# mbavaro/gnss-sdr.ru

Measured on NVIDIA B200. Metric: tracking channel*Msamples/s, higher is better.
Workload: dtype int32

## Files before the change

gnss_sdr_ru_b200/csrc/track_seg.cuh:

```cuda
#pragma once
#include "track_common.cuh"

struct __align__(16) BlockParams {
  uint32_t cph0, kph0, cinc, kinc;
  uint32_t hc0, w1, stale_idx, stale_bits;
  int mode, event;
  uint32_t wtot;
  uint32_t seg;
  double dinv;
  uint32_t kseg;
  uint32_t pad;
};
static_assert(sizeof(BlockParams) == 64, "BlockParams: four 16-byte rows");

#ifndef SEG_U2
#define SEG_U2 1
#endif
#ifndef SEG_PIN
#define SEG_PIN 0
#endif

__device__ __forceinline__ uint32_t lds_u32(uint32_t addr) {
  uint32_t t;
  asm volatile("ld.shared.u32 %0, [%1];" : "=r"(t) : "r"(addr));
  return t;
}

__device__ __forceinline__ bool seg_kinc_ok(uint32_t kinc) { return kinc >= (1u << 29) && 7ull * kinc <= (1ull << 32); }
__device__ __forceinline__ bool seg_kinc_ok16(uint32_t kinc) { return kinc >= (1u << 28) && 15ull * kinc <= (1ull << 32); }

__device__ __forceinline__ uint32_t seg_start(uint32_t m, double nk05 , double dinv) {
  const double x = fma((double)m, 4294967296.0, nk05);
  return (uint32_t)(x * dinv) + 1u;
}

struct SegBounds {
  uint32_t tile_lo, tile_hi, bits_lo, bits_hi, vlut_lo, vlut_hi;
};
template <int H>
__device__ __forceinline__ void correlate_segments(uint32_t q, uint32_t cph, uint32_t ks, const uint32_t cinc, const uint32_t kinc,
                                                   const uint32_t k7, const uint32_t hp, const int nvalid, const uint32_t vlut_lane,
                                                   const PipeK K, int &accE, int &accP, int &accL, const SegBounds bnd,
                                                   const uint32_t kseg_addr ,
                                                   const uint32_t kconst_addr ) {
  int aE = 0, aP = 0, aL = 0;
  TCHECK(0, ks < kinc || nvalid == 0);
  TCHECK(1, hp >= bnd.bits_lo && hp + 4u * (H + 1) <= bnd.bits_hi + 4u);
  uint32_t a0 = (q >> 3) & ~3u;
  TCHECK(2, a0 >= bnd.tile_lo && a0 + 8u <= bnd.tile_hi);
  uint32_t lo = lds_u32(a0), hi = lds_u32(a0 + 4);
  uint32_t t = lds_u32(hp);
  uint32_t hq = hp;
  const uint32_t hq_valid = hp + 4u * (uint32_t)nvalid;
  const uint32_t hq_end = hp + 4u * (uint32_t)H;
#if SEG_PIN
  uint32_t k7r, k1r, k2048r;
  asm volatile("ld.volatile.shared.u32 %0, [%1];" : "=r"(k7r) : "r"(kseg_addr));
  asm volatile("ld.volatile.shared.v2.u32 {%0, %1}, [%2];" : "=r"(k1r), "=r"(k2048r) : "r"(kconst_addr));
  TCHECK(0, k7r == k7 && k1r == K.k1 && k2048r == K.k2048);
#else
  const uint32_t k7r = k7, k1r = K.k1, k2048r = K.k2048;
#endif
#define SEG_BODY(tc, tn)                                                                                             \
  {                                                                                                                  \
                      \
    const uint32_t wd = __funnelshift_r(lo, hi, q);                                                                  \
            \
    uint32_t u, c;                                                                                                   \
    asm("add.cc.u32 %0, %2, %3;\n\taddc.u32 %1, 0, 0;" : "=r"(u), "=r"(c) : "r"(ks), "r"(k7r));                    \
    const uint32_t e8 = k1r - c;                                                                                     \
    ks = e8 * kinc + u;                                                                                              \
    q = e8 * 4u + (q + 28u);                                                                                         \
     \
    const uint32_t a = (q >> 3) & ~3u;                                                                               \
    TCHECK(2, a >= bnd.tile_lo && a + 8u <= bnd.tile_hi);    \
    lo = lds_u32(a);                                                                                                 \
    hi = lds_u32(a + 4);                                                                                             \
    tn = lds_u32(hq + 4u);                                                                                           \
    int v[8];                                                                                                        \
    _Pragma("unroll") for (int k = 0; k < 8; k++) {                                                                  \
                                                          \
      uint32_t sh;                                                                                                   \
      if (k == 0)                                                                                                    \
        sh = wd << 7;                                                                                                \
      else if (k == 1)                                                                                               \
        sh = wd << 3;                                                                                                \
      else                                                                                                           \
        sh = wd >> (4 * k - 7);                                                                                      \
      uint32_t ca;                                                                                                   \
      asm("lop3.b32 %0, %1, 0x780, %2, 0xEA;" : "=r"(ca) : "r"(sh), "r"(vlut_lane));   \
      const uint32_t eaddr = (cph >> 29) * k2048r + ca;            \
      TCHECK(3, eaddr >= bnd.vlut_lo && eaddr + 4u <= bnd.vlut_hi);                           \
      v[k] = (int)lds_u32(eaddr);                                                                                    \
      if (k < 7) cph += cinc;                                                                                        \
    }                                                                                                                \
    cph = e8 * cinc + cph;                                                                                           \
    const int S = (int)e8 * v[7] + (((v[0] + v[1] + v[2]) + (v[3] + v[4] + v[5])) + v[6]);                           \
    if (hq < hq_valid) {                                                                                             \
      aE += sext8(tc, 0) * S;                                                                                        \
      aP += sext8(tc, 1) * S;                                                                                        \
      aL += sext8(tc, 2) * S;                                                                                        \
    }                                                                                                                \
    hq += 4u;                                                                                                        \
  }
#if SEG_U2
  uint32_t t2;
  if (H & 1) {
    SEG_BODY(t, t2)
    t = t2;
  }
  if (H > 1) {
#pragma unroll 1
    do {
      SEG_BODY(t, t2)
      SEG_BODY(t2, t)
    } while (hq != hq_end);
  }
#else
#pragma unroll 1
  do {
    uint32_t t_next;
    SEG_BODY(t, t_next)
    t = t_next;
  } while (hq != hq_end);
#endif
#undef SEG_BODY
  accE = aE;
  accP = aP;
  accL = aL;
}

template <int H>
__device__ __forceinline__ void correlate_segments_i8(uint32_t q, uint32_t cph, uint32_t ks, const uint32_t cinc, const uint32_t kinc,
                                                      const uint32_t k7, const uint32_t hp, const int nvalid, const uint32_t lut_addr,
                                                      const PipeK K, int &accE, int &accP, int &accL, const SegBounds bnd) {
  static_assert(8 * H * 384 <= 32767, "int8 segment run: a 16-bit lane of the packed sums can overflow");
  int aE = 0, aP = 0, aL = 0;
  TCHECK(0, ks < kinc || nvalid == 0);
  TCHECK(1, hp >= bnd.bits_lo && hp + 4u * (H + 1) <= bnd.bits_hi + 4u);
  uint32_t hq = hp;
  const uint32_t hq_valid = hp + 4u * (uint32_t)nvalid;
  const uint32_t hq_end = hp + 4u * (uint32_t)H;
#pragma unroll 1
  do {
    const uint32_t a = (q >> 3) & ~3u;
    TCHECK(2, a >= bnd.tile_lo && a + 20u <= bnd.tile_hi);
    uint32_t w[5];
#pragma unroll
    for (int i = 0; i < 5; i++) w[i] = lds_u32(a + 4u * i);
    const uint32_t t = lds_u32(hq);
    uint32_t x[4];
#pragma unroll
    for (int i = 0; i < 4; i++) x[i] = __funnelshift_r(w[i], w[i + 1], q);
    uint32_t u, c;
    asm("add.cc.u32 %0, %2, %3;\n\taddc.u32 %1, 0, 0;" : "=r"(u), "=r"(c) : "r"(ks), "r"(k7));
    const uint32_t e8 = K.k1 - c;
    ks = e8 * kinc + u;
    q = e8 * 16u + (q + 112u);
    int v[8];
#pragma unroll
    for (int k = 0; k < 8; k++) {
      const int I = sext8(x[k >> 1], (k & 1) * 2), Q = sext8(x[k >> 1], (k & 1) * 2 + 1);
      uint32_t lx, ly;
      asm volatile("ld.shared.v2.u32 {%0, %1}, [%2];" : "=r"(lx), "=r"(ly) : "r"((cph >> 29) * K.k8 + lut_addr));
      v[k] = I * (int)lx + Q * (int)ly;
      if (k < 7) cph += cinc;
    }
    cph = e8 * cinc + cph;
    const int S = (int)e8 * v[7] + (((v[0] + v[1] + v[2]) + (v[3] + v[4] + v[5])) + v[6]);
    if (hq < hq_valid) {
      aE += sext8(t, 0) * S;
      aP += sext8(t, 1) * S;
      aL += sext8(t, 2) * S;
    }
    hq += 4u;
  } while (hq != hq_end);
  accE = aE;
  accP = aP;
  accL = aL;
}

template <int H>
__device__ __forceinline__ void correlate_segments16(uint32_t q, uint32_t cph, uint32_t ks, const uint32_t cinc, const uint32_t kinc,
                                                     const uint32_t k15, const uint32_t hp, const int nvalid, const uint32_t vlut_lane,
                                                     const PipeK K, int &accE, int &accP, int &accL, const SegBounds bnd) {
  int aE = 0, aP = 0, aL = 0;
  TCHECK(0, ks < kinc || nvalid == 0);
  TCHECK(1, hp >= bnd.bits_lo && hp + 4u * (H + 1) <= bnd.bits_hi + 4u);
  uint32_t hq = hp;
  const uint32_t hq_valid = hp + 4u * (uint32_t)nvalid;
  const uint32_t hq_end = hp + 4u * (uint32_t)H;
#pragma unroll 1
  do {
    const uint32_t a = (q >> 3) & ~3u;
    TCHECK(2, a >= bnd.tile_lo && a + 12u <= bnd.tile_hi);
    const uint32_t w0 = lds_u32(a), w1 = lds_u32(a + 4), w2 = lds_u32(a + 8);
    const uint32_t t = lds_u32(hq);
    const uint32_t wd[2] = {__funnelshift_r(w0, w1, q), __funnelshift_r(w1, w2, q)};
    uint32_t u, c;
    asm("add.cc.u32 %0, %2, %3;\n\taddc.u32 %1, 0, 0;" : "=r"(u), "=r"(c) : "r"(ks), "r"(k15));
    const uint32_t e16 = K.k1 - c;
    ks = e16 * kinc + u;
    q = e16 * 4u + (q + 60u);
    int S = 0;
#pragma unroll
    for (int half = 0; half < 2; half++) {
      int v[8];
#pragma unroll
      for (int k = 0; k < 8; k++) {
        uint32_t sh;
        if (k == 0)
          sh = wd[half] << 7;
        else if (k == 1)
          sh = wd[half] << 3;
        else
          sh = wd[half] >> (4 * k - 7);
        uint32_t ca;
        asm("lop3.b32 %0, %1, 0x780, %2, 0xEA;" : "=r"(ca) : "r"(sh), "r"(vlut_lane));
        const uint32_t eaddr = (cph >> 29) * K.k2048 + ca;
        TCHECK(3, eaddr >= bnd.vlut_lo && eaddr + 4u <= bnd.vlut_hi);
        v[k] = (int)lds_u32(eaddr);
        if (half == 0 || k < 7) cph += cinc;
      }
      S += ((v[0] + v[1] + v[2]) + (v[3] + v[4] + v[5])) + v[6] + (half == 0 ? v[7] : (int)e16 * v[7]);
    }
    cph = e16 * cinc + cph;
    if (hq < hq_valid) {
      aE += sext8(t, 0) * S;
      aP += sext8(t, 1) * S;
      aL += sext8(t, 2) * S;
    }
    hq += 4u;
  } while (hq != hq_end);
  accE = aE;
  accP = aP;
  accL = aL;
}

struct SampleCtx {
  uint32_t cph0, kph0, cinc, kinc, hc0, w1, stale_idx;
  const uint8_t *tile;
  const uint32_t *tbl;
  const uint2 *lut;
  int fmt;
};
__device__ __forceinline__ void eval_sample(const SampleCtx &c, int i, int (&sumA)[6], int (&sumB)[6], bool &anyB) {
  const unsigned long long ki = (unsigned long long)c.kph0 + (unsigned long long)i * c.kinc;
  const uint32_t wb = (uint32_t)(ki >> 32);
  const bool inA = wb < c.w1;
  const uint32_t rel = wb - c.w1;
  const uint32_t hh = inA ? c.hc0 + wb : (rel == 0 ? c.stale_idx : rel);
  TCHECK(5, hh < SMEM_TBL);
  const uint32_t t = c.tbl[hh];
  int I, Q;
  load_sample(c.tile, c.fmt, i, I, Q);
  const uint2 ab = c.lut[(c.cph0 + (uint32_t)i * c.cinc) >> 29];
  const int v = I * (int)ab.x + Q * (int)ab.y;
  int vi, vq;
  unpack_lanes(v, vi, vq);
  const int cE = sext8(t, 0), cP = sext8(t, 1), cL = sext8(t, 2);
  if (inA) {
    sumA[0] += cL * vi; sumA[1] += cL * vq; sumA[2] += cP * vi;
    sumA[3] += cP * vq; sumA[4] += cE * vi; sumA[5] += cE * vq;
  } else {
    sumB[0] += cL * vi; sumB[1] += cL * vq; sumB[2] += cP * vi;
    sumB[3] += cP * vq; sumB[4] += cE * vi; sumB[5] += cE * vq;
    anyB = true;
  }
}

template <int NT, int H, int SLOTS = 8, bool I8 = false>
__device__ __forceinline__ void seg_block(const BlockParams &p, const SampleCtx &sc, const uint32_t tile_addr, const uint32_t tbl_addr,
                                          const uint32_t alias_addr, const uint32_t vlut_lane, const PipeK K, const int nsamp,
                                          const int ptid, int (&sumA)[6], int (&sumB)[6], bool &anyB, const SegBounds bnd_in,
                                          const uint32_t kseg_addr = 0, const uint32_t kconst_addr = 0) {
  constexpr int STEP = NT == 96 ? 7 : 1;
  const int tid = (ptid * STEP) % NT;
  const uint32_t wtot = p.wtot, w1 = p.w1;
  const uint32_t NF = wtot > 0 ? wtot - 1 : 0;
  constexpr uint32_t OWNED = (uint32_t)(NT - 1) * H;
  const double nk05 = -(double)p.kph0 - 0.5;
  uint32_t m0, nv;
  if (tid < NT - 1) {
    const uint32_t first = (uint32_t)tid * H;
    m0 = 1 + first;
    nv = NF > first ? min(NF - first, (uint32_t)H) : 0u;
    if (m0 < w1 && w1 < m0 + nv) nv = w1 - m0;
  } else {
    m0 = 1;
    nv = 0;
    if (w1 >= 2) {
      const uint32_t ts = (w1 - 2) / H, first = ts * H;
      const uint32_t end = 1 + first + (NF > first ? min(NF - first, (uint32_t)H) : 0u);
      if (ts < (uint32_t)(NT - 1) && w1 < end) {
        m0 = w1;
        nv = end - w1;
      }
    }
  }
  if (nv == 0) m0 = 1;
  const bool clsB = m0 >= w1;
  uint32_t hp;
  if (clsB) {
    const uint32_t rel = m0 - w1;
    hp = rel == 0 ? alias_addr : tbl_addr + 4u * rel;
  } else
    hp = tbl_addr + 4u * (p.hc0 + m0);
  const uint32_t s = seg_start(m0, nk05, p.dinv);
  SegBounds bnd = bnd_in;
  if (clsB && m0 == w1) {
    bnd.bits_lo = alias_addr;
    bnd.bits_hi = alias_addr + 4u * 48u;
  }
  TCHECK(4, nv == 0 || s + (uint32_t)(SLOTS - 1) * nv <= (uint32_t)nsamp);
  int pE, pP, pL;
  if constexpr (I8)
    correlate_segments_i8<H>(8u * tile_addr + 16u * s, p.cph0 + s * p.cinc, p.kph0 + s * p.kinc, p.cinc, p.kinc, 7u * p.kinc, hp, (int)nv,
                             vlut_lane, K, pE, pP, pL, bnd);
  else if constexpr (SLOTS == 16)
    correlate_segments16<H>(8u * tile_addr + 4u * s, p.cph0 + s * p.cinc, p.kph0 + s * p.kinc, p.cinc, p.kinc, 15u * p.kinc, hp, (int)nv,
                            vlut_lane, K, pE, pP, pL, bnd);
  else
    correlate_segments<H>(8u * tile_addr + 4u * s, p.cph0 + s * p.cinc, p.kph0 + s * p.kinc, p.cinc, p.kinc, 7u * p.kinc, hp, (int)nv,
                          vlut_lane, K, pE, pP, pL, bnd, kseg_addr, kconst_addr);
  {
    int v[6];
    unpack_lanes(pL, v[0], v[1]);
    unpack_lanes(pP, v[2], v[3]);
    unpack_lanes(pE, v[4], v[5]);
    if (clsB) {
#pragma unroll
      for (int q = 0; q < 6; q++) sumB[q] += v[q];
      anyB |= nv != 0;
    } else {
#pragma unroll
      for (int q = 0; q < 6; q++) sumA[q] += v[q];
    }
  }
  if (ptid < 32) {
    const uint32_t head_end = wtot == 0 ? (uint32_t)nsamp : min(seg_start(1, nk05, p.dinv), (uint32_t)nsamp);
    const uint32_t mt = 1 + min(NF, OWNED);
    const uint32_t tail_start = mt > wtot ? (uint32_t)nsamp : min(seg_start(mt, nk05, p.dinv), (uint32_t)nsamp);
    const uint32_t total = head_end + ((uint32_t)nsamp - tail_start);
    for (uint32_t e = (uint32_t)ptid; e < total; e += 32) {
      const uint32_t i = e < head_end ? e : tail_start + (e - head_end);
      eval_sample(sc, (int)i, sumA, sumB, anyB);
    }
  }
}

template <int NT>
__device__ __forceinline__ void generic_block(const SampleCtx &sc, const int nsamp, const int tid, int (&sumA)[6], int (&sumB)[6],
                                              bool &anyB) {
  for (int i = tid; i < nsamp; i += NT) eval_sample(sc, i, sumA, sumB, anyB);
}
```

gnss_sdr_ru_b200/csrc/track_ws.cuh:

```cuda
#pragma once
#include "track_common.cuh"
#include "track_seg.cuh"

__device__ __forceinline__ void mbar_arrive(uint64_t *bar) {
  asm volatile("mbarrier.arrive.shared::cta.b64 _, [%0];" ::"r"(smem_u32(bar)) : "memory");
}
__device__ __forceinline__ int warp_sum(int v) { return __reduce_add_sync(0xffffffffu, v); }

__device__ __forceinline__ bool block_is_event(const StepParams &sp, const TrackArgs &a, bool last) {
  if (sp.mode != MODE_FAST || last) return true;
  const unsigned long long nk = (unsigned long long)a.nsamp * sp.kinc;
  const unsigned long long kend = (unsigned long long)sp.kph0 + nk;
  const uint32_t wtot = (uint32_t)(kend >> 32);
  const unsigned long long wnext = ((unsigned long long)(uint32_t)kend + nk) >> 32;
  const bool next_fast = wnext < (unsigned long long)(sp.w1 - wtot) + sp.slew_dump && (wnext + 40) < SMEM_TBL;
  const bool quiet = wtot < sp.w1 && !(sp.tic_count >= 0 && sp.tic_count < a.nsamp) && next_fast;
  return !quiet;
}
__device__ __forceinline__ void advance_quiet(StepParams &sp, const TrackArgs &a) {
  const unsigned long long n = (unsigned long long)a.nsamp;
  const unsigned long long kend = (unsigned long long)sp.kph0 + n * sp.kinc;
  const unsigned long long cend = (unsigned long long)sp.cph0 + n * sp.cinc;
  const uint32_t wtot = (uint32_t)(kend >> 32);
  sp.kph0 = (uint32_t)kend;
  sp.cph0 = (uint32_t)cend;
  sp.hc0 += wtot;
  sp.w1 -= wtot;
  sp.cyc_pending += (uint32_t)(cend >> 32);
  if (sp.tic < (long long)n) {
    sp.tic_count = (int)sp.tic;
    sp.tic += a.cfg.tic_ref - (long long)n;
  } else {
    sp.tic_count = -1;
    sp.tic -= (long long)n;
  }
}

typedef unsigned long long SchedSlot;
struct SchedQueue {
  unsigned head, tail, total, nchan;
  long long slice_blocks;
  long long *tic;
  int32_t *dumpcnt;
  SchedSlot *slots;
};

__global__ void sched_init_kernel(SchedQueue *q, unsigned nchan, unsigned nslices, long long slice_blocks, long long *tic,
                                  int32_t *dumpcnt, SchedSlot *slots) {
  const unsigned i = blockIdx.x * blockDim.x + threadIdx.x;
  if (i == 0) {
    q->head = 0;
    q->tail = nchan;
    q->total = nchan * nslices;
    q->nchan = nchan;
    q->slice_blocks = slice_blocks;
    q->tic = tic;
    q->dumpcnt = dumpcnt;
    q->slots = slots;
  }
  if (i < nchan) {
    slots[i] = (unsigned long long)i | ((unsigned long long)i << 32);
    dumpcnt[i] = 0;
    tic[i] = 0;
  }
}

template <class T>
__device__ __forceinline__ void copy_in_cg(T &dst, const T *src) {
  static_assert(sizeof(T) % 4 == 0, "word copy");
  const int *s4 = reinterpret_cast<const int *>(src);
  int *d4 = reinterpret_cast<int *>(&dst);
  for (int i = 0; i < (int)(sizeof(T) / 4); i++) d4[i] = __ldcg(s4 + i);
}

template <int MINB, int FMT, int CT, int SEGH = 0>
__global__ void __launch_bounds__(CT + 32, MINB) track_ws_kernel(const TrackArgs a, const int tile_bytes) {
  constexpr int WS_CORR_THREADS = CT;
  constexpr int SPT = SEGH > 0 ? 32 : 8192 / CT;
  static_assert(SEGH > 0 || CT * SPT == 8192, "fixed-run form: CT threads x SPT samples cover the largest block");
  constexpr int WS_THREADS = WS_CORR_THREADS + 32;
  constexpr int fmt = FMT;
  constexpr bool packed_native = FMT == GNSSB200_FMT_PACKED2;
  static_assert(SEGH == 0 || FMT == GNSSB200_FMT_PACKED2 || FMT == GNSSB200_FMT_INT8_IQ, "the segment form reads packed or int8 I,Q samples");
  __shared__ ChanShared cs;
  __shared__ BlockParams params[2];
  __shared__ uint2 lut[8];
  __shared__ uint32_t tbl[SMEM_TBL];
  __shared__ uint32_t alias_tbl[2][48];
  __shared__ __align__(16) int totals[12];
  __shared__ __align__(8) uint32_t kconst[2];
  __shared__ __align__(8) uint64_t dfull[2], pfull[2], empty[2], tfull;
  extern __shared__ __align__(128) uint8_t tiles[];
  uint8_t *vlut_raw = tiles + 2 * (size_t)tile_bytes;
  if (SEGH > 0) vlut_raw += (2048u - (smem_u32(vlut_raw) & 2047u)) & 2047u;
  uint32_t *vlut = reinterpret_cast<uint32_t *>(vlut_raw);

  __shared__ int s_item;
  const int tid = threadIdx.x, lane = tid & 31, warp = tid >> 5;
  const size_t blk_bytes = bytes_for(fmt, a.nsamp);
  constexpr int CTRL = 0, CTRL_WARP = 0;
  const int ctid = tid - 32;
  SchedQueue *const wq = a.sched;
  fill_lo_lut(lut);
  if (tid == 0) {
    kconst[0] = a.k1;
    kconst[1] = a.k2048;
  }
  if (packed_native) {
    for (int i = tid; i < 128 * 32; i += WS_THREADS) {
      const int e = i >> 5, ph = e >> 4, code = e & 15;
      const int I = sample_val((uint32_t)code), Q = sample_val((uint32_t)code >> 2);
      const int ival = lo_i(ph) * I + lo_q(ph) * Q, qval = lo_q(ph) * I - lo_i(ph) * Q;
      vlut[i] = (uint32_t)(ival + 65536 * qval);
    }
  }
  const bool queued = wq != nullptr;
  if (queued && tid == CTRL) {
    const unsigned ticket = atomicAdd(&wq->head, 1u);
    volatile SchedSlot *slot = wq->slots + ticket % wq->nchan;
    unsigned long long v;
    while ((unsigned)(v = *slot) != ticket) __nanosleep(100);
    __threadfence();
    s_item = (int)(v >> 32);
    TCHECK(6, (unsigned)s_item < wq->total);
  }
  __syncthreads();
  const int item = queued ? s_item : (int)blockIdx.x;
  const int nchan = queued ? (int)wq->nchan : (int)gridDim.x;
  const long long slice_blocks = queued ? wq->slice_blocks : a.nblocks;
  const int chan_id = item % nchan, slice = item / nchan;
  const int s = a.first_stream + chan_id / NCH, ch = chan_id % NCH;
  gnssb200_rx *rx = a.rx + s;
  const int tbl_prn = __ldcg(&rx->reg_write[ch << 3]);
  const long long slice_first = (long long)slice * slice_blocks;
  const long long nblocks = min(slice_blocks, a.nblocks - slice_first);
  const uint8_t *stream_base = a.d_if + (size_t)s * a.stride + (size_t)slice_first * blk_bytes;

  if (tid < 12) totals[tid] = 0;
  for (int i = tid; i < SMEM_TBL; i += WS_THREADS) {
    long long f = code_table_base(tbl_prn) + i;
    tbl[i] = (code_has_fast_row(tbl_prn) && f < TABLE_ENTRIES) ? a.code_table[f] : 0u;
  }
  if (tid < 96) {
    const int t = tid % 48;
    long long f = code_table_base(tbl_prn) + t;
    alias_tbl[tid / 48][t] = (code_has_fast_row(tbl_prn) && f < TABLE_ENTRIES) ? a.code_table[f] : 0u;
  }
  __syncthreads();
  const int b8 = ch << 3;
  StepParams sp;
  long long first_block = 0;
  long long loaded = -1;
  if (tid == CTRL) {
    copy_in_cg(cs.k, &rx->chan[ch]);
    copy_in_cg(cs.g, &rx->corr[ch]);
    cs.r.w_prn = __ldcg(&rx->reg_write[b8]);
    cs.r.w_carr_hi = __ldcg(&rx->reg_write[b8 + 3]);
    cs.r.w_carr_lo = __ldcg(&rx->reg_write[b8 + 4]);
    cs.r.w_code_hi = __ldcg(&rx->reg_write[b8 + 5]);
    cs.r.w_code_lo = __ldcg(&rx->reg_write[b8 + 6]);
    cs.r.w_epoch = __ldcg(&rx->reg_write[b8 + 7]);
    cs.r.w_slew = __ldcg(&rx->reg_write[b8 + 0x84]);
    for (int j = 0; j < 8; j++) cs.r.r_meas[j] = __ldcg(&rx->reg_read[b8 + j]);
    for (int j = 0; j < 6; j++) cs.r.r_acc[j] = __ldcg(&rx->reg_read[b8 + 0x84 + j]);
    const int prev_flags = slice > 0 ? __ldcg(&a.chan_flags[s * NCH + ch]) : 0;
    cs.tic = slice > 0 ? __ldcg(&wq->tic[chan_id]) : rx->tic;
    cs.dumped_last = prev_flags & 1;
    cs.halted = (prev_flags >> 1) & 1;
    cs.dump_count = a.dump_count ? __ldcg(&a.dump_count[s * NCH + ch]) : (slice > 0 ? __ldcg(&wq->dumpcnt[chan_id]) : 0);
    first_block = rx->blocks_done + slice_first;
#ifdef TRACK_CHECK
    TCHECK(7, (atomicOr(&a.chan_flags[s * NCH + ch], 4) & 4) == 0);
#endif
    sp.stale_bits = 0;
    if (nblocks > 0 && !rx->halted && !cs.halted) {
      prepare_block(cs, sp, a, tbl_prn);
      if (sp.mode == MODE_FAST) sp.stale_bits = tbl[sp.stale_idx];
    } else
      sp.mode = MODE_STOP;
    mbar_init(&dfull[0], 1);
    mbar_init(&dfull[1], 1);
    mbar_init(&pfull[0], 1);
    mbar_init(&pfull[1], 1);
    mbar_init(&empty[0], WS_CORR_THREADS / 32);
    mbar_init(&empty[1], WS_CORR_THREADS / 32);
    mbar_init(&tfull, WS_CORR_THREADS / 32);
    asm volatile("fence.mbarrier_init.release.cluster;" ::: "memory");
    asm volatile("fence.proxy.async.shared::cta;" ::: "memory");
    if (sp.mode == MODE_FAST || sp.mode == MODE_SERIAL) {
      mbar_expect_tx(&dfull[0], (uint32_t)blk_bytes);
      tma_load_1d(tiles, stream_base, (uint32_t)blk_bytes, &dfull[0]);
      loaded = 0;
    }
  }
  __syncthreads();

  if (warp == CTRL_WARP) {
    if (lane != 0) return;
    uint32_t inv_of = 0;
    double dinv = 0.0;
    auto publish = [&](int slot, const StepParams &sp, bool event) {
      BlockParams &p = params[slot];
      p.cph0 = sp.cph0; p.kph0 = sp.kph0; p.cinc = sp.cinc; p.kinc = sp.kinc;
      p.hc0 = sp.hc0; p.w1 = sp.w1; p.stale_idx = sp.stale_idx; p.stale_bits = sp.stale_bits;
      p.mode = sp.mode; p.event = event ? 1 : 0;
      if constexpr (SEGH > 0) {
        if (sp.mode == MODE_FAST) {
          const uint32_t form = seg_kinc_ok(sp.kinc) ? 1u : ((packed_native && seg_kinc_ok16(sp.kinc)) ? 2u : 0u);
          const bool ok = form != 0;
          if (ok && sp.kinc != inv_of) {
            dinv = 1.0 / (double)sp.kinc;
            inv_of = sp.kinc;
          }
          p.wtot = (uint32_t)(((unsigned long long)sp.kph0 + (unsigned long long)a.nsamp * sp.kinc) >> 32);
          p.seg = form;
          p.dinv = dinv;
          p.kseg = 7u * sp.kinc;
        }
      }
      alias_tbl[slot][0] = sp.stale_bits;
      mbar_arrive(&pfull[slot]);
    };
    bool event = block_is_event(sp, a, nblocks <= 1);
#ifdef EXP_ALL_QUIET
    if (sp.mode == MODE_FAST && nblocks > 1) event = false;
#endif
    publish(0, sp, event);
    uint32_t ev_phase = 0;
#ifdef TRACK_PROFILE
    long long c_twait = 0, c_fin = 0, c_words = 0, c_params = 0, c_rest = 0, c_ewait = 0, c_quiet = 0, n_ev = 0, n_q = 0, c_acc = 0, c_prep = 0, c_cls = 0;
#define CP(var) { long long _c = clock64(); var += _c - _t; _t = _c; }
#else
#define CP(var)
#endif
    for (long long b = 0; b < nblocks; b++) {
      if (sp.mode == MODE_STOP) break;
#ifdef TRACK_PROFILE
      long long _t = clock64();
#endif
      const bool last = b + 1 == nblocks;
      const int slot = (int)(b & 1), nslot = slot ^ 1;
      if (!last) {
        if (b >= 1) mbar_wait(&empty[nslot], (uint32_t)(((b - 1) >> 1) & 1));
        if (sp.mode != MODE_IDLE) {
          mbar_expect_tx(&dfull[nslot], (uint32_t)blk_bytes);
          tma_load_1d(tiles + (size_t)nslot * tile_bytes, stream_base + (size_t)(b + 1) * blk_bytes, (uint32_t)blk_bytes, &dfull[nslot]);
          loaded = b + 1;
        }
      }
      CP(c_ewait)
      if (!event) {
        advance_quiet(sp, a);
        event = block_is_event(sp, a, b + 2 == nblocks);
#ifdef EXP_ALL_QUIET
        if (sp.mode == MODE_FAST && b + 2 != nblocks) event = false;
#endif
        publish(nslot, sp, event);
#ifdef TRACK_PROFILE
        n_q++;
#endif
        CP(c_quiet)
        continue;
      }
#ifdef TRACK_PROFILE
      n_ev++;
#endif
      cs.tic = sp.tic;
      cs.g.carrier_cycle += sp.cyc_pending;
      const int was_mode = sp.mode;
      if (was_mode == MODE_FAST) {
        finalize_state(cs, sp, a.nsamp);
        if (!last) prepare_block_state(cs, sp, a);
      }
      CP(c_fin)
#ifdef EXP_EARLY_PUBLISH
      bool early = false;
      ChRegs saved_r = cs.r;
      if (was_mode == MODE_FAST && !last) {
        StepParams t = sp;
        prepare_block_regs(cs, t, a, tbl_prn);
        t.stale_bits = t.mode == MODE_FAST ? tbl[t.stale_idx] : 0u;
        publish(nslot, t, block_is_event(t, a, b + 2 == nblocks));
        early = true;
      }
#endif
      if (was_mode == MODE_FAST) {
        int A[6], B[6];
        mbar_wait(&tfull, ev_phase);
        ev_phase ^= 1;
        CP(c_twait)
        const int4 t0 = *reinterpret_cast<const int4 *>(&totals[0]);
        const int4 t1 = *reinterpret_cast<const int4 *>(&totals[4]);
        const int4 t2 = *reinterpret_cast<const int4 *>(&totals[8]);
        A[0] = t0.x; A[1] = t0.y; A[2] = t0.z; A[3] = t0.w; A[4] = t1.x; A[5] = t1.y;
        B[0] = t1.z; B[1] = t1.w; B[2] = t2.x; B[3] = t2.y; B[4] = t2.z; B[5] = t2.w;
        const int4 z = make_int4(0, 0, 0, 0);
        *reinterpret_cast<int4 *>(&totals[0]) = z;
        *reinterpret_cast<int4 *>(&totals[4]) = z;
        *reinterpret_cast<int4 *>(&totals[8]) = z;
        finalize_acc(cs, A, B);
        CP(c_acc)
      } else if (was_mode == MODE_SERIAL) {
        mbar_wait(&dfull[slot], (uint32_t)((b >> 1) & 1));
        {
          const StepParams p_tmp = sp;
          serial_block(cs, p_tmp, a.code_table, fmt, a.nsamp, tiles + (size_t)slot * tile_bytes);
        }
        if (!last) prepare_block_state(cs, sp, a);
      } else
        cs.dumped_last = 0;
      int st_in = -1;
      bool isr = false;
      if (cs.dumped_last && a.run_isr) {
        if (dev_gpsisr_words(cs.k, cs.r, a.cfg, st_in))
          cs.halted = 1;
        else
          isr = true;
      }
      CP(c_words)
#ifdef EXP_EARLY_PUBLISH
      if (early) {
        cs.r.w_carr_hi = saved_r.w_carr_hi; cs.r.w_carr_lo = saved_r.w_carr_lo; cs.r.w_code_hi = saved_r.w_code_hi;
        cs.r.w_code_lo = saved_r.w_code_lo; cs.r.w_slew = saved_r.w_slew;
        cs.halted = 0;
      }
#endif
      if (cs.halted || was_mode == MODE_IDLE)
        sp.mode = MODE_STOP;
      else if (!last) {
        prepare_block_regs(cs, sp, a, tbl_prn);
        sp.stale_bits = sp.mode == MODE_FAST ? tbl[sp.stale_idx] : 0u;
      }
      CP(c_prep)
      if (!last) {
        event = block_is_event(sp, a, b + 2 == nblocks);
        CP(c_cls)
#ifdef EXP_EARLY_PUBLISH
        if (!early)
#endif
        publish(nslot, sp, event);
      }
      CP(c_params)
      if (isr) dev_gpsisr_rest(cs.k, cs.r, a.cfg, st_in);
      if (cs.dumped_last && !cs.halted && a.dumps && cs.dump_count < a.dump_cap) {
        gnssb200_dump *out = &a.dumps[((size_t)s * NCH + ch) * a.dump_cap + cs.dump_count];
        int4 q0, q1, q2;
        q0.x = (int)(first_block + b);
        q0.y = (int)(uint16_t)(int16_t)ch | ((int)(uint16_t)(int16_t)cs.k.state << 16);
        q0.z = cs.r.r_acc[0];
        q0.w = cs.r.r_acc[1];
        q1.x = cs.r.r_acc[2];
        q1.y = cs.r.r_acc[3];
        q1.z = cs.r.r_acc[4];
        q1.w = cs.r.r_acc[5];
        q2.x = (cs.r.w_carr_hi << 16) + cs.r.w_carr_lo;
        q2.y = (cs.r.w_code_hi << 16) + cs.r.w_code_lo;
        q2.z = (int)(uint16_t)(int16_t)cs.k.n_freq | ((int)(uint16_t)(int16_t)cs.k.codes << 16);
        q2.w = cs.r.w_slew;
        int4 *o4 = reinterpret_cast<int4 *>(out);
        o4[0] = q0;
        o4[1] = q1;
        o4[2] = q2;
        cs.dump_count++;
      }
      if (!last && sp.mode != MODE_STOP) apply_epoch_load(cs);
      CP(c_rest)
    }
#ifdef TRACK_PROFILE
    if (blockIdx.x == 0 && n_ev && n_q)
      printf("control lane: %lld quiet blocks: slot wait+TMA %lld, classify+publish %lld | %lld event blocks: totals wait %lld finalize %lld isr words %lld params+publish %lld rest %lld (cycles each)\n",
             n_q, c_ewait / (n_q + n_ev), c_quiet / n_q, n_ev, c_twait / n_ev, c_fin / n_ev, c_words / n_ev, c_params / n_ev, c_rest / n_ev);
    if (blockIdx.x == 0 && n_ev)
      printf("   after the totals: read+accumulators %lld, isr words %lld, prepare params %lld, classify %lld, publish %lld\n", c_acc / n_ev, c_words / n_ev, c_prep / n_ev,
             c_cls / n_ev, c_params / n_ev);
#endif
    if (loaded >= 0) mbar_wait(&dfull[loaded & 1], (uint32_t)((loaded >> 1) & 1));
    rx->chan[ch] = cs.k;
    rx->corr[ch] = cs.g;
    rx->reg_write[b8 + 3] = cs.r.w_carr_hi;
    rx->reg_write[b8 + 4] = cs.r.w_carr_lo;
    rx->reg_write[b8 + 5] = cs.r.w_code_hi;
    rx->reg_write[b8 + 6] = cs.r.w_code_lo;
    rx->reg_write[b8 + 7] = cs.r.w_epoch;
    rx->reg_write[b8 + 0x84] = cs.r.w_slew;
    for (int q = 1; q < 8; q++) rx->reg_read[b8 + q] = cs.r.r_meas[q];
    for (int q = 0; q < 6; q++) rx->reg_read[b8 + 0x84 + q] = cs.r.r_acc[q];
    a.chan_flags[s * NCH + ch] = (cs.dumped_last ? 1 : 0) | (cs.halted ? 2 : 0);
    if (a.dump_count) a.dump_count[s * NCH + ch] = cs.dump_count;
    if (queued) {
      if (!a.dump_count) wq->dumpcnt[chan_id] = cs.dump_count;
      wq->tic[chan_id] = cs.tic;
    }
    const unsigned next_item = (unsigned)item + (unsigned)nchan;
    if (queued && next_item < wq->total) {
      __threadfence();
      const unsigned t = atomicAdd(&wq->tail, 1u);
      atomicExch(wq->slots + t % wq->nchan, (unsigned long long)t | ((unsigned long long)next_item << 32));
    }
    return;
  }

  const int i0 = ctid * SPT;
  const bool live = i0 < a.nsamp;
  const uint32_t vlut_lane = smem_u32(vlut) + 4u * (uint32_t)lane;
  int carry[6] = {0, 0, 0, 0, 0, 0};
#ifdef TRACK_PROFILE
  long long t_pw = 0, t_dw = 0, t_corr = 0, t_red = 0, t_all = -clock64(), nb = 0;
#endif
  for (long long b = 0; b < nblocks; b++) {
    const int slot = (int)(b & 1);
    const uint32_t par = (uint32_t)((b >> 1) & 1);
#ifdef TRACK_PROFILE
    long long _t = clock64();
    nb++;
#endif
    mbar_wait(&pfull[slot], par);
    CP(t_pw)
    const uint4 p0 = reinterpret_cast<const uint4 *>(&params[slot])[0];
    const uint4 p1 = reinterpret_cast<const uint4 *>(&params[slot])[1];
    const int2 p2 = reinterpret_cast<const int2 *>(&params[slot])[4];
    const int mode = p2.x;
    const bool event = p2.y != 0;
    if (mode == MODE_STOP) break;
    if (mode == MODE_FAST) {
      const uint32_t cph0 = p0.x, kph0 = p0.y, cinc = p0.z, kinc = p0.w;
      const uint32_t hc0 = p1.x, w1 = p1.y, stale_idx = p1.z, stale_bits = p1.w;
      const uint8_t *tile = tiles + (size_t)slot * tile_bytes;
      mbar_wait(&dfull[slot], par);
      CP(t_dw)
      int sumA[6] = {0, 0, 0, 0, 0, 0}, sumB[6] = {0, 0, 0, 0, 0, 0};
      bool anyB = false;
      if constexpr (SEGH > 0) {
        BlockParams bp;
        bp.cph0 = cph0; bp.kph0 = kph0; bp.cinc = cinc; bp.kinc = kinc;
        bp.hc0 = hc0; bp.w1 = w1; bp.stale_idx = stale_idx; bp.stale_bits = stale_bits;
        const uint2 p3 = reinterpret_cast<const uint2 *>(&params[slot])[5];
        bp.wtot = p3.x;
        bp.seg = p3.y;
        bp.dinv = params[slot].dinv;
        const SampleCtx sc{cph0, kph0, cinc, kinc, hc0, w1, stale_idx, tile, tbl, lut, fmt};
        const SegBounds bnd{smem_u32(tile), smem_u32(tile) + (uint32_t)tile_bytes + (packed_native ? 64u : 224u), smem_u32(tbl), smem_u32(tbl) + 4u * SMEM_TBL,
#ifdef TRACK_CHECK_SELFTEST
                            smem_u32(vlut), smem_u32(vlut) + 64u * 32u * 4u};
#else
                            smem_u32(vlut), smem_u32(vlut) + 128u * 32u * 4u};
#endif
        constexpr int SEGH16 = (SEGH * 8 + 15) / 16;
        bool done = false;
        if constexpr (packed_native) {
          if (bp.seg == 1) {
            seg_block<CT, SEGH>(bp, sc, smem_u32(tile), smem_u32(tbl), smem_u32(alias_tbl[slot]), vlut_lane,
                                PipeK{a.k1, a.k8, a.k128, a.k2048}, a.nsamp, ctid, sumA, sumB, anyB, bnd, smem_u32(&params[slot].kseg),
                                smem_u32(kconst));
            done = true;
          } else if (bp.seg == 2) {
            seg_block<CT, SEGH16, 16>(bp, sc, smem_u32(tile), smem_u32(tbl), smem_u32(alias_tbl[slot]), vlut_lane,
                                      PipeK{a.k1, a.k8, a.k128, a.k2048}, a.nsamp, ctid, sumA, sumB, anyB, bnd);
            done = true;
          }
        } else {
          if (bp.seg == 1) {
            seg_block<CT, SEGH, 8, true>(bp, sc, smem_u32(tile), smem_u32(tbl), smem_u32(alias_tbl[slot]), smem_u32(lut),
                                         PipeK{a.k1, a.k8, a.k128, a.k2048}, a.nsamp, ctid, sumA, sumB, anyB, bnd);
            done = true;
          }
        }
        if (!done) generic_block<CT>(sc, a.nsamp, ctid, sumA, sumB, anyB);
      } else {
        uint32_t cur[SPT / 2];
        uint32_t pk[SPT / 8];
        if (live && packed_native) {
          const uint32_t *pp = reinterpret_cast<const uint32_t *>(tile + (i0 >> 1));
#pragma unroll
          for (int q = 0; q < SPT / 8; q++) pk[q] = pp[q];
        } else if (live) {
          load_chunk<SPT, true>(tile, fmt, i0, a.nsamp, true, nullptr, cur);
        }
        const int i1 = live ? min(i0 + SPT, a.nsamp) : i0 + 1;
        const unsigned long long k0 = (unsigned long long)kph0 + (unsigned long long)i0 * kinc;
        const uint32_t w_start = (uint32_t)(k0 >> 32);
        const uint32_t w_lastb = (uint32_t)(((unsigned long long)kph0 + (unsigned long long)(i1 - 1) * kinc) >> 32);
        const bool allA = !live || w_lastb < w1, allB = live && w_start >= w1;
        uint32_t h, hl;
        if (allB) {
          h = w_start - w1;
          hl = (h == 0) ? stale_idx : h;
        } else {
          h = hc0 + w_start;
          hl = h;
        }
        int pE = 0, pP = 0, pL = 0;
        const bool stale_start = allB && h == 0;
        if (live && packed_native)
          correlate_chunk_packed<SPT>(pk, cph0 + (uint32_t)i0 * cinc, (uint32_t)k0, cinc, kinc, stale_start ? alias_tbl[slot] : tbl, h,
                                      stale_start ? stale_bits : tbl[hl], vlut_lane, PipeK{a.k1, a.k8, a.k128, a.k2048}, pE, pP, pL);
        else if (live)
          correlate_chunk<SPT>(cur, cph0 + (uint32_t)i0 * cinc, (uint32_t)k0, cinc, kinc, stale_start ? alias_tbl[slot] : tbl, h,
                               stale_start ? stale_bits : tbl[hl], lut, pE, pP, pL);
        const bool straddle = !allA && !allB;
        if (!straddle && live) {
          int v[6];
          unpack_lanes(pL, v[0], v[1]);
          unpack_lanes(pP, v[2], v[3]);
          unpack_lanes(pE, v[4], v[5]);
          if (allA) {
#pragma unroll
            for (int q = 0; q < 6; q++) sumA[q] += v[q];
          } else {
#pragma unroll
            for (int q = 0; q < 6; q++) sumB[q] += v[q];
          }
        }
        unsigned m = __ballot_sync(0xffffffffu, straddle);
        while (m) {
          const int src = __ffs(m) - 1;
          m &= m - 1;
          const int si0 = __shfl_sync(0xffffffffu, i0, src);
          for (int i = si0 + lane; i < min(si0 + SPT, a.nsamp); i += 32) {
            const unsigned long long ki = (unsigned long long)kph0 + (unsigned long long)i * kinc;
            const uint32_t wb = (uint32_t)(ki >> 32);
            const bool inA = wb < w1;
            const uint32_t rel = wb - w1;
            const uint32_t hh = inA ? hc0 + wb : (rel == 0 ? stale_idx : rel);
            const uint32_t t = tbl[hh];
            int I, Q;
            load_sample(tile, fmt, i, I, Q);
            const uint2 ab = lut[(cph0 + (uint32_t)i * cinc) >> 29];
            const int v = I * (int)ab.x + Q * (int)ab.y;
            int vi, vq;
            unpack_lanes(v, vi, vq);
            const int cE = sext8(t, 0), cP = sext8(t, 1), cL = sext8(t, 2);
            if (inA) {
              sumA[0] += cL * vi; sumA[1] += cL * vq; sumA[2] += cP * vi;
              sumA[3] += cP * vq; sumA[4] += cE * vi; sumA[5] += cE * vq;
            } else {
              sumB[0] += cL * vi; sumB[1] += cL * vq; sumB[2] += cP * vi;
              sumB[3] += cP * vq; sumB[4] += cE * vi; sumB[5] += cE * vq;
            }
          }
        }
        anyB |= !allA;
      }
      CP(t_corr)
      if (!event) {
#pragma unroll
        for (int q = 0; q < 6; q++) carry[q] += sumA[q];
      } else {
        const bool warpB = __any_sync(0xffffffffu, anyB);
        int va = 0, vb = 0;
#pragma unroll
        for (int q = 0; q < 6; q++) {
          const int ra = warp_sum(sumA[q] + carry[q]);
          carry[q] = 0;
          if (lane == q) va = ra;
        }
        if (warpB) {
#pragma unroll
          for (int q = 0; q < 6; q++) {
            const int rb = warp_sum(sumB[q]);
            if (lane == q) vb = rb;
          }
        }
        if (lane < 6) {
          atomicAdd(&totals[lane], va);
          if (warpB) atomicAdd(&totals[6 + lane], vb);
        }
      }
    }
    __syncwarp();
    if (lane == 0) {
      if (event && mode == MODE_FAST) mbar_arrive(&tfull);
      mbar_arrive(&empty[slot]);
    }
    CP(t_red)
  }
#ifdef TRACK_PROFILE
  t_all += clock64();
  if (blockIdx.x == 0 && (tid == 0 || tid == 133) && nb)
    printf("correlator tid %d: per block: params wait %lld  data wait %lld  load+correlate+post %lld  reduce/arrive %lld  total %lld\n", tid, t_pw / nb, t_dw / nb,
           t_corr / nb, t_red / nb, t_all / nb);
#endif
}
```

Baseline: 1.960 million.

## Split segment correlation into two interleaved independent chains per thread

Each thread's segment run is split into two halves whose starting phase is computed independently with seg_start, and the two dependency chains are stepped in an interleaved loop to expose instruction-level parallelism through the serial carry/phase recurrence. The SEG_PIN shared-memory constant pinning path and the kseg/kconst plumbing are removed, the thread permutation stride for 96-thread blocks changes from 7 to 23, and the queue re-enqueue logic now reads the channel from s_item. This adds register pressure and an extra seg_start division per thread in exchange for shorter critical paths.

```diff
diff --git a/gnss_sdr_ru_b200/csrc/track_seg.cuh b/gnss_sdr_ru_b200/csrc/track_seg.cuh
--- a/gnss_sdr_ru_b200/csrc/track_seg.cuh
+++ b/gnss_sdr_ru_b200/csrc/track_seg.cuh
@@ -8,17 +8,9 @@
   uint32_t wtot;
   uint32_t seg;
   double dinv;
-  uint32_t kseg;
-  uint32_t pad;
+  uint32_t pad[2];
 };
 static_assert(sizeof(BlockParams) == 64, "BlockParams: four 16-byte rows");
-
-#ifndef SEG_U2
-#define SEG_U2 1
-#endif
-#ifndef SEG_PIN
-#define SEG_PIN 0
-#endif
 
 __device__ __forceinline__ uint32_t lds_u32(uint32_t addr) {
   uint32_t t;
@@ -34,97 +26,80 @@
   return (uint32_t)(x * dinv) + 1u;
 }
 
+struct SegChain {
+  uint32_t q, cph, ks, lo, hi;
+};
 struct SegBounds {
   uint32_t tile_lo, tile_hi, bits_lo, bits_hi, vlut_lo, vlut_hi;
 };
+__device__ __forceinline__ void seg_step(SegChain &c, const uint32_t ha, const uint32_t ha_valid, const uint32_t cinc, const uint32_t kinc,
+                                         const uint32_t k7, const uint32_t vlut_lane, const PipeK K, int &aE, int &aP, int &aL,
+                                         const SegBounds &bnd) {
+  const uint32_t wd = __funnelshift_r(c.lo, c.hi, c.q);
+  const uint32_t t = lds_u32(ha);
+  uint32_t u, cy;
+  asm("add.cc.u32 %0, %2, %3;\n\taddc.u32 %1, 0, 0;" : "=r"(u), "=r"(cy) : "r"(c.ks), "r"(k7));
+  const uint32_t e8 = K.k1 - cy;
+  c.ks = e8 * kinc + u;
+  c.q = e8 * 4u + (c.q + 28u);
+  const uint32_t a = (c.q >> 3) & ~3u;
+  TCHECK(2, a >= bnd.tile_lo && a + 8u <= bnd.tile_hi);
+  c.lo = lds_u32(a);
+  c.hi = lds_u32(a + 4);
+  int v[8];
+#pragma unroll
+  for (int k = 0; k < 8; k++) {
+    uint32_t sh;
+    if (k == 0)
+      sh = wd << 7;
+    else if (k == 1)
+      sh = wd << 3;
+    else
+      sh = wd >> (4 * k - 7);
+    uint32_t ca;
+    asm("lop3.b32 %0, %1, 0x780, %2, 0xEA;" : "=r"(ca) : "r"(sh), "r"(vlut_lane));
+    const uint32_t eaddr = (c.cph >> 29) * K.k2048 + ca;
+    TCHECK(3, eaddr >= bnd.vlut_lo && eaddr + 4u <= bnd.vlut_hi);
+    v[k] = (int)lds_u32(eaddr);
+    if (k < 7) c.cph += cinc;
+  }
+  c.cph = e8 * cinc + c.cph;
+  const int S = (int)e8 * v[7] + (((v[0] + v[1] + v[2]) + (v[3] + v[4] + v[5])) + v[6]);
+  if (ha < ha_valid) {
+    aE += sext8(t, 0) * S;
+    aP += sext8(t, 1) * S;
+    aL += sext8(t, 2) * S;
+  }
+}
+
 template <int H>
-__device__ __forceinline__ void correlate_segments(uint32_t q, uint32_t cph, uint32_t ks, const uint32_t cinc, const uint32_t kinc,
-                                                   const uint32_t k7, const uint32_t hp, const int nvalid, const uint32_t vlut_lane,
-                                                   const PipeK K, int &accE, int &accP, int &accL, const SegBounds bnd,
-                                                   const uint32_t kseg_addr ,
-                                                   const uint32_t kconst_addr ) {
+__device__ __forceinline__ void correlate_segments(SegChain a, SegChain b, const uint32_t cinc, const uint32_t kinc, const uint32_t k7,
+                                                   const uint32_t hp, const int nvalid, const uint32_t vlut_lane, const PipeK K,
+                                                   int &accE, int &accP, int &accL, const SegBounds bnd) {
+  constexpr int HA = (H + 1) / 2, HB = H / 2;
+  static_assert(HB >= 1, "two chains need two segments");
   int aE = 0, aP = 0, aL = 0;
-  TCHECK(0, ks < kinc || nvalid == 0);
-  TCHECK(1, hp >= bnd.bits_lo && hp + 4u * (H + 1) <= bnd.bits_hi + 4u);
-  uint32_t a0 = (q >> 3) & ~3u;
-  TCHECK(2, a0 >= bnd.tile_lo && a0 + 8u <= bnd.tile_hi);
-  uint32_t lo = lds_u32(a0), hi = lds_u32(a0 + 4);
-  uint32_t t = lds_u32(hp);
+  TCHECK(0, (a.ks < kinc && b.ks < kinc) || nvalid == 0);
+  TCHECK(1, hp >= bnd.bits_lo && hp + 4u * H <= bnd.bits_hi);
+  const uint32_t a0 = (a.q >> 3) & ~3u, b0 = (b.q >> 3) & ~3u;
+  TCHECK(2, a0 >= bnd.tile_lo && a0 + 8u <= bnd.tile_hi && b0 >= bnd.tile_lo && b0 + 8u <= bnd.tile_hi);
+  a.lo = lds_u32(a0);
+  a.hi = lds_u32(a0 + 4);
+  b.lo = lds_u32(b0);
+  b.hi = lds_u32(b0 + 4);
   uint32_t hq = hp;
   const uint32_t hq_valid = hp + 4u * (uint32_t)nvalid;
-  const uint32_t hq_end = hp + 4u * (uint32_t)H;
-#if SEG_PIN
-  uint32_t k7r, k1r, k2048r;
-  asm volatile("ld.volatile.shared.u32 %0, [%1];" : "=r"(k7r) : "r"(kseg_addr));
-  asm volatile("ld.volatile.shared.v2.u32 {%0, %1}, [%2];" : "=r"(k1r), "=r"(k2048r) : "r"(kconst_addr));
-  TCHECK(0, k7r == k7 && k1r == K.k1 && k2048r == K.k2048);
-#else
-  const uint32_t k7r = k7, k1r = K.k1, k2048r = K.k2048;
-#endif
-#define SEG_BODY(tc, tn)                                                                                             \
-  {                                                                                                                  \
-                      \
-    const uint32_t wd = __funnelshift_r(lo, hi, q);                                                                  \
-            \
-    uint32_t u, c;                                                                                                   \
-    asm("add.cc.u32 %0, %2, %3;\n\taddc.u32 %1, 0, 0;" : "=r"(u), "=r"(c) : "r"(ks), "r"(k7r));                    \
-    const uint32_t e8 = k1r - c;                                                                                     \
-    ks = e8 * kinc + u;                                                                                              \
-    q = e8 * 4u + (q + 28u);                                                                                         \
-     \
-    const uint32_t a = (q >> 3) & ~3u;                                                                               \
-    TCHECK(2, a >= bnd.tile_lo && a + 8u <= bnd.tile_hi);    \
-    lo = lds_u32(a);                                                                                                 \
-    hi = lds_u32(a + 4);                                                                                             \
-    tn = lds_u32(hq + 4u);                                                                                           \
-    int v[8];                                                                                                        \
-    _Pragma("unroll") for (int k = 0; k < 8; k++) {                                                                  \
-                                                          \
-      uint32_t sh;                                                                                                   \
-      if (k == 0)                                                                                                    \
-        sh = wd << 7;                                                                                                \
-      else if (k == 1)                                                                                               \
-        sh = wd << 3;                                                                                                \
-      else                                                                                                           \
-        sh = wd >> (4 * k - 7);                                                                                      \
-      uint32_t ca;                                                                                                   \
-      asm("lop3.b32 %0, %1, 0x780, %2, 0xEA;" : "=r"(ca) : "r"(sh), "r"(vlut_lane));   \
-      const uint32_t eaddr = (cph >> 29) * k2048r + ca;            \
-      TCHECK(3, eaddr >= bnd.vlut_lo && eaddr + 4u <= bnd.vlut_hi);                           \
-      v[k] = (int)lds_u32(eaddr);                                                                                    \
-      if (k < 7) cph += cinc;                                                                                        \
-    }                                                                                                                \
-    cph = e8 * cinc + cph;                                                                                           \
-    const int S = (int)e8 * v[7] + (((v[0] + v[1] + v[2]) + (v[3] + v[4] + v[5])) + v[6]);                           \
-    if (hq < hq_valid) {                                                                                             \
-      aE += sext8(tc, 0) * S;                                                                                        \
-      aP += sext8(tc, 1) * S;                                                                                        \
-      aL += sext8(tc, 2) * S;                                                                                        \
-    }                                                                                                                \
-    hq += 4u;                                                                                                        \
-  }
-#if SEG_U2
-  uint32_t t2;
+  const uint32_t hq_end = hp + 4u * (uint32_t)HA;
   if (H & 1) {
-    SEG_BODY(t, t2)
-    t = t2;
-  }
-  if (H > 1) {
-#pragma unroll 1
-    do {
-      SEG_BODY(t, t2)
-      SEG_BODY(t2, t)
-    } while (hq != hq_end);
-  }
-#else
+    seg_step(a, hq, hq_valid, cinc, kinc, k7, vlut_lane, K, aE, aP, aL, bnd);
+    hq += 4u;
+  }
 #pragma unroll 1
   do {
-    uint32_t t_next;
-    SEG_BODY(t, t_next)
-    t = t_next;
+    seg_step(a, hq, hq_valid, cinc, kinc, k7, vlut_lane, K, aE, aP, aL, bnd);
+    seg_step(b, hq + 4u * HB, hq_valid, cinc, kinc, k7, vlut_lane, K, aE, aP, aL, bnd);
+    hq += 4u;
   } while (hq != hq_end);
-#endif
-#undef SEG_BODY
   accE = aE;
   accP = aP;
   accL = aL;
@@ -272,9 +247,8 @@
 template <int NT, int H, int SLOTS = 8, bool I8 = false>
 __device__ __forceinline__ void seg_block(const BlockParams &p, const SampleCtx &sc, const uint32_t tile_addr, const uint32_t tbl_addr,
                                           const uint32_t alias_addr, const uint32_t vlut_lane, const PipeK K, const int nsamp,
-                                          const int ptid, int (&sumA)[6], int (&sumB)[6], bool &anyB, const SegBounds bnd_in,
-                                          const uint32_t kseg_addr = 0, const uint32_t kconst_addr = 0) {
-  constexpr int STEP = NT == 96 ? 7 : 1;
+                                          const int ptid, int (&sumA)[6], int (&sumB)[6], bool &anyB, const SegBounds bnd_in) {
+  constexpr int STEP = NT == 96 ? 23 : 1;
   const int tid = (ptid * STEP) % NT;
   const uint32_t wtot = p.wtot, w1 = p.w1;
   const uint32_t NF = wtot > 0 ? wtot - 1 : 0;
@@ -320,9 +294,12 @@
   else if constexpr (SLOTS == 16)
     correlate_segments16<H>(8u * tile_addr + 4u * s, p.cph0 + s * p.cinc, p.kph0 + s * p.kinc, p.cinc, p.kinc, 15u * p.kinc, hp, (int)nv,
                             vlut_lane, K, pE, pP, pL, bnd);
-  else
-    correlate_segments<H>(8u * tile_addr + 4u * s, p.cph0 + s * p.cinc, p.kph0 + s * p.kinc, p.cinc, p.kinc, 7u * p.kinc, hp, (int)nv,
-                          vlut_lane, K, pE, pP, pL, bnd, kseg_addr, kconst_addr);
+  else {
+    const uint32_t sb = seg_start(m0 + (H + 1) / 2, nk05, p.dinv);
+    correlate_segments<H>(SegChain{8u * tile_addr + 4u * s, p.cph0 + s * p.cinc, p.kph0 + s * p.kinc, 0u, 0u},
+                          SegChain{8u * tile_addr + 4u * sb, p.cph0 + sb * p.cinc, p.kph0 + sb * p.kinc, 0u, 0u}, p.cinc, p.kinc,
+                          7u * p.kinc, hp, (int)nv, vlut_lane, K, pE, pP, pL, bnd);
+  }
   {
     int v[6];
     unpack_lanes(pL, v[0], v[1]);
diff --git a/gnss_sdr_ru_b200/csrc/track_ws.cuh b/gnss_sdr_ru_b200/csrc/track_ws.cuh
--- a/gnss_sdr_ru_b200/csrc/track_ws.cuh
+++ b/gnss_sdr_ru_b200/csrc/track_ws.cuh
@@ -88,7 +88,6 @@
   __shared__ uint32_t tbl[SMEM_TBL];
   __shared__ uint32_t alias_tbl[2][48];
   __shared__ __align__(16) int totals[12];
-  __shared__ __align__(8) uint32_t kconst[2];
   __shared__ __align__(8) uint64_t dfull[2], pfull[2], empty[2], tfull;
   extern __shared__ __align__(128) uint8_t tiles[];
   uint8_t *vlut_raw = tiles + 2 * (size_t)tile_bytes;
@@ -102,10 +101,6 @@
   const int ctid = tid - 32;
   SchedQueue *const wq = a.sched;
   fill_lo_lut(lut);
-  if (tid == 0) {
-    kconst[0] = a.k1;
-    kconst[1] = a.k2048;
-  }
   if (packed_native) {
     for (int i = tid; i < 128 * 32; i += WS_THREADS) {
       const int e = i >> 5, ph = e >> 4, code = e & 15;
@@ -215,7 +210,6 @@
           p.wtot = (uint32_t)(((unsigned long long)sp.kph0 + (unsigned long long)a.nsamp * sp.kinc) >> 32);
           p.seg = form;
           p.dinv = dinv;
-          p.kseg = 7u * sp.kinc;
         }
       }
       alias_tbl[slot][0] = sp.stale_bits;
@@ -388,14 +382,15 @@
     a.chan_flags[s * NCH + ch] = (cs.dumped_last ? 1 : 0) | (cs.halted ? 2 : 0);
     if (a.dump_count) a.dump_count[s * NCH + ch] = cs.dump_count;
     if (queued) {
-      if (!a.dump_count) wq->dumpcnt[chan_id] = cs.dump_count;
-      wq->tic[chan_id] = cs.tic;
-    }
-    const unsigned next_item = (unsigned)item + (unsigned)nchan;
-    if (queued && next_item < wq->total) {
-      __threadfence();
-      const unsigned t = atomicAdd(&wq->tail, 1u);
-      atomicExch(wq->slots + t % wq->nchan, (unsigned long long)t | ((unsigned long long)next_item << 32));
+      const unsigned qitem = *reinterpret_cast<volatile int *>(&s_item), qchan = qitem % (unsigned)nchan;
+      if (!a.dump_count) wq->dumpcnt[qchan] = cs.dump_count;
+      wq->tic[qchan] = cs.tic;
+      const unsigned next_item = qitem + (unsigned)nchan;
+      if (next_item < wq->total) {
+        __threadfence();
+        const unsigned t = atomicAdd(&wq->tail, 1u);
+        atomicExch(wq->slots + t % wq->nchan, (unsigned long long)t | ((unsigned long long)next_item << 32));
+      }
     }
     return;
   }
@@ -450,8 +445,7 @@
         if constexpr (packed_native) {
           if (bp.seg == 1) {
             seg_block<CT, SEGH>(bp, sc, smem_u32(tile), smem_u32(tbl), smem_u32(alias_tbl[slot]), vlut_lane,
-                                PipeK{a.k1, a.k8, a.k128, a.k2048}, a.nsamp, ctid, sumA, sumB, anyB, bnd, smem_u32(&params[slot].kseg),
-                                smem_u32(kconst));
+                                PipeK{a.k1, a.k8, a.k128, a.k2048}, a.nsamp, ctid, sumA, sumB, anyB, bnd);
             done = true;
           } else if (bp.seg == 2) {
             seg_block<CT, SEGH16, 16>(bp, sc, smem_u32(tile), smem_u32(tbl), smem_u32(alias_tbl[slot]), vlut_lane,
```

Measured after the change: 1.921 million, median of 6. 2.0% lower.
